# xqtr/PySpecSDR

Hardware: AMD Instinct MI355X
Metric: IQ MSamples/sec end-to-end (FFT+dB+FM demod) (higher is better)
Workload: dtype complex64 IQ / f64 FFT + dB + post-process + FIR + IIR / dB rows stored as f32 / int16 PCM

## Files before the change

pyspecsdr_amd/csrc/pss_fft_r16.h:

```cpp
#pragma once
#include <hip/hip_runtime.h>

#include "pss_npf32.h"
#include "pss_device.h"

namespace pss_r16 {

#ifdef PSS_EXP_NOFMA
__device__ __forceinline__ double2 cmul(double2 a, double2 b) { return make_double2(a.x * b.x - a.y * b.y, a.x * b.y + a.y * b.x); }
__device__ __forceinline__ double power_of(double2 X) { return X.x * X.x + X.y * X.y + 1e-10; }
#else
__device__ __forceinline__ double2 cmul(double2 a, double2 b) { return make_double2(fma(a.x, b.x, -(a.y * b.y)), fma(a.x, b.y, a.y * b.x)); }
__device__ __forceinline__ double power_of(double2 X) { return fma(X.x, X.x, fma(X.y, X.y, 1e-10)); }
#endif
__device__ __forceinline__ double2 cadd(double2 a, double2 b) { return make_double2(a.x + b.x, a.y + b.y); }
__device__ __forceinline__ double2 csub(double2 a, double2 b) { return make_double2(a.x - b.x, a.y - b.y); }

constexpr int brev(int i, int bits)
{
    int r = 0;
    for (int b = 0; b < bits; b++) r |= ((i >> b) & 1) << (bits - 1 - b);
    return r;
}
constexpr int ilog2c(int n) { return n <= 1 ? 0 : 1 + ilog2c(n >> 1); }

template <int J, int LEN>
__device__ __forceinline__ double2 twc(double2 a)
{
    constexpr int j16 = (J * (16 / LEN)) & 15;
    constexpr double C1 = 0.92387953251128673848, S1 = 0.38268343236508978178, H = 0.70710678118654752440;
    if constexpr (j16 == 0) return a;
    else if constexpr (j16 == 4) return make_double2(a.y, -a.x);
    else if constexpr (j16 == 8) return make_double2(-a.x, -a.y);
    else if constexpr (j16 == 12) return make_double2(-a.y, a.x);
    else if constexpr (j16 == 2) return make_double2((a.x + a.y) * H, (a.y - a.x) * H);
    else if constexpr (j16 == 6) return make_double2((a.y - a.x) * H, -(a.x + a.y) * H);
    else if constexpr (j16 == 1) return cmul(a, make_double2(C1, -S1));
    else if constexpr (j16 == 3) return cmul(a, make_double2(S1, -C1));
    else if constexpr (j16 == 5) return cmul(a, make_double2(-S1, -C1));
    else if constexpr (j16 == 7) return cmul(a, make_double2(-C1, -S1));
    else return a;
}

template <int R, int LEN = R, int BASE = 0>
struct Dif {
    template <int J>
    static __device__ __forceinline__ void bf(double2 (&v)[R])
    {
        if constexpr (J < LEN / 2) {
            double2 a = v[BASE + J], b = v[BASE + J + LEN / 2];
            v[BASE + J] = cadd(a, b);
            v[BASE + J + LEN / 2] = twc<J, LEN>(csub(a, b));
            bf<J + 1>(v);
        }
    }
    static __device__ __forceinline__ void run(double2 (&v)[R])
    {
        if constexpr (LEN >= 2) {
            bf<0>(v);
            Dif<R, LEN / 2, BASE>::run(v);
            Dif<R, LEN / 2, BASE + LEN / 2>::run(v);
        }
    }
};

template <int R>
__device__ __forceinline__ void fft_reg(double2 (&v)[R])
{
    if constexpr (R > 1) Dif<R>::run(v);
}

static __constant__ double2 DB_TAB[97] = {
    {0x1.5555555555555p+0, -0x1.ffbfc2bbc7802p-4},
    {0x1.51d07eae2f815p+0, -0x1.ed50a4a26eafbp-4},
    {0x1.4e5e0a72f0539p+0, -0x1.db11ed766abf2p-4},
    {0x1.4afd6a052bf5bp+0, -0x1.c902a19e65114p-4},
    {0x1.47ae147ae147bp+0, -0x1.b721cd17157e3p-4},
    {0x1.446f86562d9fbp+0, -0x1.a56e8325f5c87p-4},
    {0x1.4141414141414p+0, -0x1.93e7de0fc3e7fp-4},
    {0x1.3e22cbce4a902p+0, -0x1.828cfed29a212p-4},
    {0x1.3b13b13b13b14p+0, -0x1.715d0ce367afdp-4},
    {0x1.3813813813814p+0, -0x1.605735ee985f4p-4},
    {0x1.3521cfb2b78c1p+0, -0x1.4f7aad9bbcbaep-4},
    {0x1.323e34a2b10bfp+0, -0x1.3ec6ad5407866p-4},
    {0x1.2f684bda12f68p+0, -0x1.2e3a740b7800dp-4},
    {0x1.2c9fb4d812ca0p+0, -0x1.1dd5460c8b170p-4},
    {0x1.29e4129e4129ep+0, -0x1.0d966cc6500f8p-4},
    {0x1.27350b8812735p+0, -0x1.fafa6d397efdbp-5},
    {0x1.2492492492492p+0, -0x1.db11ed766abf1p-5},
    {0x1.21fb78121fb78p+0, -0x1.bb7209d1e24e4p-5},
    {0x1.1f7047dc11f70p+0, -0x1.9c197abf00dd3p-5},
    {0x1.1cf06ada2811dp+0, -0x1.7d070145f4fd8p-5},
    {0x1.1a7b9611a7b96p+0, -0x1.5e3966b7e9294p-5},
    {0x1.1811811811812p+0, -0x1.3faf7c6630614p-5},
    {0x1.15b1e5f75270dp+0, -0x1.21681b5c8c213p-5},
    {0x1.135c81135c811p+0, -0x1.0362241e638eap-5},
    {0x1.1111111111111p+0, -0x1.cb38fccd8bfdap-6},
    {0x1.0ecf56be69c90p+0, -0x1.902c31d62a847p-6},
    {0x1.0c9714fbcda3bp+0, -0x1.559bd2406c3c1p-6},
    {0x1.0a6810a6810a7p+0, -0x1.1b85d6044e9bbp-6},
    {0x1.0842108421084p+0, -0x1.c3d0837784c3ap-7},
    {0x1.0624dd2f1a9fcp+0, -0x1.51824c7587eb5p-7},
    {0x1.0410410410410p+0, -0x1.c03a80ae5e038p-8},
    {0x1.0204081020408p+0, -0x1.be76bd77b4fb5p-9},
    {0x1.0000000000000p+0, 0x0.0p+0},
    {0x1.fc07f01fc07f0p-1, 0x1.bafd47221ed34p-9},
    {0x1.f81f81f81f820p-1, 0x1.b9476a4fcd0f3p-8},
    {0x1.f44659e4a4271p-1, 0x1.49b085144368ep-7},
    {0x1.f07c1f07c1f08p-1, 0x1.b5e908eb13789p-7},
    {0x1.ecc07b301ecc0p-1, 0x1.10a83a8446c7fp-6},
    {0x1.e9131abf0b767p-1, 0x1.45f4f5acb8be3p-6},
    {0x1.e573ac901e574p-1, 0x1.7adc3df3b1ff3p-6},
    {0x1.e1e1e1e1e1e1ep-1, 0x1.af5f92b00e611p-6},
    {0x1.de5d6e3f8868ap-1, 0x1.e3806acbd0593p-6},
    {0x1.dae6076b981dbp-1, 0x1.0ba01a816ffffp-5},
    {0x1.d77b654b82c34p-1, 0x1.25502c0fc3148p-5},
    {0x1.d41d41d41d41dp-1, 0x1.3ed1199a5e427p-5},
    {0x1.d0cb58f6ec074p-1, 0x1.58238eeb353dcp-5},
    {0x1.cd85689039b0bp-1, 0x1.71483427d2a97p-5},
    {0x1.ca4b3055ee191p-1, 0x1.8a3fadeb847f4p-5},
    {0x1.c71c71c71c71cp-1, 0x1.a30a9d609efedp-5},
    {0x1.c3f8f01c3f8f0p-1, 0x1.bba9a058dfd85p-5},
    {0x1.c0e070381c0e0p-1, 0x1.d41d5164facb7p-5},
    {0x1.bdd2b899406f7p-1, 0x1.ec6647eb5880bp-5},
    {0x1.bacf914c1bad0p-1, 0x1.02428c1f08014p-4},
    {0x1.b7d6c3dda338bp-1, 0x1.0e3d29d81165fp-4},
    {0x1.b4e81b4e81b4fp-1, 0x1.1a23445501814p-4},
    {0x1.b2036406c80d9p-1, 0x1.25f5215eb594ap-4},
    {0x1.af286bca1af28p-1, 0x1.31b3055c4711ap-4},
    {0x1.ac5701ac5701bp-1, 0x1.3d5d335c53178p-4},
    {0x1.a98ef606a63bep-1, 0x1.48f3ed1df48f9p-4},
    {0x1.a6d01a6d01a6dp-1, 0x1.5477731973e85p-4},
    {0x1.a41a41a41a41ap-1, 0x1.5fe80488af4fep-4},
    {0x1.a16d3f97a4b02p-1, 0x1.6b45df6f3e2c8p-4},
    {0x1.9ec8e951033d9p-1, 0x1.769140a2526fdp-4},
    {0x1.9c2d14ee4a102p-1, 0x1.81ca63d05a448p-4},
    {0x1.999999999999ap-1, 0x1.8cf183886480bp-4},
    {0x1.970e4f80cb872p-1, 0x1.9806d9414a20cp-4},
    {0x1.948b0fcd6e9e0p-1, 0x1.a30a9d609efebp-4},
    {0x1.920fb49d0e229p-1, 0x1.adfd07416be06p-4},
    {0x1.8f9c18f9c18fap-1, 0x1.b8de4d3ab3d97p-4},
    {0x1.8d3018d3018d3p-1, 0x1.c3aea4a5c6effp-4},
    {0x1.8acb90f6bf3aap-1, 0x1.ce6e41e463da3p-4},
    {0x1.886e5f0abb04ap-1, 0x1.d91d5866aa99ap-4},
    {0x1.8618618618618p-1, 0x1.e3bc1ab0e1a00p-4},
    {0x1.83c977ab2beddp-1, 0x1.ee4aba610f205p-4},
    {0x1.8181818181818p-1, 0x1.f8c9683468191p-4},
    {0x1.7f405fd017f40p-1, 0x1.019c2a064b487p-3},
    {0x1.7d05f417d05f4p-1, 0x1.06cbd67a6c3b7p-3},
    {0x1.7ad2208e0ecc3p-1, 0x1.0bf3d0937c41dp-3},
    {0x1.78a4c8178a4c8p-1, 0x1.11142f0811357p-3},
    {0x1.767dce434a9b1p-1, 0x1.162d082ac9d10p-3},
    {0x1.745d1745d1746p-1, 0x1.1b3e71ec94f7ap-3},
    {0x1.724287f46debcp-1, 0x1.204881dee8777p-3},
    {0x1.702e05c0b8170p-1, 0x1.254b4d35e7d3dp-3},
    {0x1.6e1f76b4337c7p-1, 0x1.2a46e8ca7ba29p-3},
    {0x1.6c16c16c16c17p-1, 0x1.2f3b691c5a000p-3},
    {0x1.6a13cd1537290p-1, 0x1.3428e2540096ep-3},
    {0x1.6816816816817p-1, 0x1.390f6844a0b82p-3},
    {0x1.661ec6a5122f9p-1, 0x1.3def0e6dfdf85p-3},
    {0x1.642c8590b2164p-1, 0x1.42c7e7fe3fc02p-3},
    {0x1.623fa77016240p-1, 0x1.479a07d3b6410p-3},
    {0x1.6058160581606p-1, 0x1.4c65807e93337p-3},
    {0x1.5e75bb8d015e7p-1, 0x1.512a644296c3ep-3},
    {0x1.5c9882b931057p-1, 0x1.55e8c518b10f9p-3},
    {0x1.5ac056b015ac0p-1, 0x1.5aa0b4b0988fap-3},
    {0x1.58ed2308158edp-1, 0x1.5f52447255c93p-3},
    {0x1.571ed3c506b3ap-1, 0x1.63fd857fc49bap-3},
    {0x1.5555555555555p-1, 0x1.68a288b60b7fdp-3}};

__device__ __forceinline__ double db64_of_exact(double pw, const double2 *tab = DB_TAB)
{
    const unsigned hi = (unsigned)__double2hiint(pw), lo = (unsigned)__double2loint(pw);
    const bool up = (hi & 0xfffffu) >= 0x80000u;
    const int e = (int)(hi >> 20) - 1023 + (up ? 1 : 0);
    const double z = __hiloint2double((int)((hi & 0xfffffu) | (up ? 0x3fe00000u : 0x3ff00000u)), (int)lo);
    const int i = (int)fma(z, 128.0, -95.5);
    const double2 tc = tab[i];
    const double r = fma(z, tc.x, -1.0);
    double p = fma(r, -0x1.5555555555555p-3, 0x1.999999999999ap-3);
    p = fma(p, r, -0.25);
    p = fma(p, r, 0x1.5555555555555p-2);
    p = fma(p, r, -0.5);
    p = fma(p, r, 1.0);
    double res = fma(p * r, 0x1.bcb7b1526e50ep-2, tc.y);
    res = fma((double)e, 0x1.34413509f79ffp-2, res);
    return hi >= 0x7ff00000u ? pw : 10.0 * res;
}

__device__ __forceinline__ float db_of_exact(double pw, const double2 *tab = DB_TAB)
{
    const unsigned hi = (unsigned)__double2hiint(pw), lo = (unsigned)__double2loint(pw);
    const bool up = (hi & 0xfffffu) >= 0x80000u;
    const int e = (int)(hi >> 20) - 1023 + (up ? 1 : 0);
    const double z = __hiloint2double((int)((hi & 0xfffffu) | (up ? 0x3fe00000u : 0x3ff00000u)), (int)lo);
    const int i = (int)fma(z, 128.0, -95.5);
    const double2 tc = tab[i];
    const double r = fma(z, tc.x, -1.0);
    double p = fma(r, -0x1.5555555555555p-3, 0x1.999999999999ap-3);
    p = fma(p, r, -0.25);
    p = fma(p, r, 0x1.5555555555555p-2);
    p = fma(p, r, -0.5);
    p = fma(p, r, 1.0);
    double res = fma(p * r, 0x1.bcb7b1526e50ep-2, tc.y);
    res = fma((double)e, 0x1.34413509f79ffp-2, res);
    const float out = (float)(10.0 * res);
    return hi >= 0x7ff00000u ? (float)pw : out;
}

__device__ __forceinline__ float db_of_fast(double pw)
{
    const float t = (float)(pw - 1.0);
    const float far = 3.0102999566398120f * __log2f((float)pw);
    const float s = t * __builtin_amdgcn_rcpf(2.0f + t);
    const float s2 = s * s;
#ifdef PSS_EXP_NOFMA
    const float p = s * (2.0f + s2 * (0.66666667f + s2 * (0.4f + s2 * (0.28571429f + s2 * 0.22222222f))));
#else
    const float p = s * fmaf(s2, fmaf(s2, fmaf(s2, fmaf(s2, 0.22222222f, 0.28571429f), 0.4f), 0.66666667f), 2.0f);
#endif
    return fabsf(t) < 0.25f ? 4.342944819032518f * p : far;
}

constexpr int FLAG_SCAN_EXACT = 1, FLAG_DB_EXACT = 2;
__device__ __forceinline__ float db_of(double pw, int flags = 0, const double2 *tab = DB_TAB)
{
    return (flags & FLAG_DB_EXACT) ? db_of_exact(pw, tab) : db_of_fast(pw);
}

typedef unsigned v2u_t __attribute__((ext_vector_type(2)));
__device__ __forceinline__ __amdgpu_buffer_rsrc_t make_rsrc(const void *p, unsigned bytes)
{
    return __builtin_amdgcn_make_buffer_rsrc(const_cast<void *>(p), 0, (int)bytes, 0x00020000);
}
__device__ __forceinline__ float2 buf_load_f2(__amdgpu_buffer_rsrc_t r, int voff, int soff)
{
    const v2u_t v = __builtin_amdgcn_raw_buffer_load_b64(r, voff, soff, 0);
    return make_float2(__uint_as_float(v.x), __uint_as_float(v.y));
}
__device__ __forceinline__ double buf_load_f64(__amdgpu_buffer_rsrc_t r, int voff, int soff)
{
    const v2u_t v = __builtin_amdgcn_raw_buffer_load_b64(r, voff, soff, 0);
    return __hiloint2double((int)v.y, (int)v.x);
}
__device__ __forceinline__ void buf_store_f32(__amdgpu_buffer_rsrc_t r, int voff, int soff, float x)
{
    __builtin_amdgcn_raw_buffer_store_b32(__float_as_uint(x), r, voff, soff, 0);
}
__device__ __forceinline__ void buf_store_f64(__amdgpu_buffer_rsrc_t r, int voff, int soff, double x)
{
    v2u_t v;
    v.x = (unsigned)__double2loint(x);
    v.y = (unsigned)__double2hiint(x);
    __builtin_amdgcn_raw_buffer_store_b64(v, r, voff, soff, 0);
}

constexpr int DPP_NEXT_LANE = 0x134;

template <int LOG_R3>
struct Cfg {
    static constexpr int R3 = 1 << LOG_R3;
    static constexpr int T = 16 * R3;
    static constexpr int N = 16 * T;
    static constexpr int FPW = 256 / T;
#ifdef PSS_EXP_OLDPAD
    static constexpr int E1_STRIDE = T + 4;
    static constexpr int E2_STRIDE = 256 + 2;
    static constexpr int TW2S = 16;
#else
    static constexpr int E1_STRIDE = T + (R3 == 1 ? 4 : R3 % 16);
    static constexpr int E2_STRIDE = 256 + (R3 == 1 ? 2 : R3 <= 8 ? 8 / R3 : 1);
    static constexpr int TW2S = 17;
#endif
    static constexpr int TW2 = R3 * TW2S;
    static __device__ __forceinline__ int tw2_slot(int i) { return (i / 16) * TW2S + (i % 16); }
    static constexpr int EX = (16 * E1_STRIDE > R3 * E2_STRIDE) ? 16 * E1_STRIDE : R3 * E2_STRIDE;
    static constexpr size_t LDS = (size_t)FPW * EX * sizeof(double2) + (size_t)TW2 * sizeof(double2);
};

template <bool WAVE_LOCAL>
__device__ __forceinline__ void frame_sync()
{
    if constexpr (WAVE_LOCAL) {
        __builtin_amdgcn_fence(__ATOMIC_RELEASE, "wavefront");
        __builtin_amdgcn_wave_barrier();
        __builtin_amdgcn_fence(__ATOMIC_ACQUIRE, "wavefront");
    } else {
        __syncthreads();
    }
}

template <int LOG_R3, bool WAVE_LOCAL = false, class Emit>
__device__ __forceinline__ void r16_core(double2 (&v)[16], double2 *ex, const double2 (&tw1)[16], const double2 *tw2,
                                         int t, Emit emit)
{
    using C = Cfg<LOG_R3>;
    constexpr int R3 = C::R3, T = C::T;
    const int k2s = t / R3, m1s = t % R3;
    fft_reg<16>(v);
#pragma unroll
    for (int k2 = 0; k2 < 16; k2++) {
        double2 y = v[brev(k2, 4)];
        if (k2) y = cmul(y, tw1[k2]);
        ex[k2 * C::E1_STRIDE + t] = y;
    }
    frame_sync<WAVE_LOCAL>();
#pragma unroll
    for (int m2 = 0; m2 < 16; m2++) v[m2] = ex[k2s * C::E1_STRIDE + m1s + R3 * m2];
    frame_sync<WAVE_LOCAL>();
#ifndef PSS_EXP_TW2_AT_USE
    constexpr int TWD = 4;
    const double2 *twp = tw2 + m1s * C::TW2S;
    double2 tq[TWD];
    if constexpr (R3 > 1) {
#pragma unroll
        for (int d = 0; d < TWD; d++) tq[d] = twp[1 + d];
        __builtin_amdgcn_sched_barrier(0);
    }
#endif
    fft_reg<16>(v);
#ifdef PSS_EXP_TW2_AT_USE
#pragma unroll
    for (int j2 = 0; j2 < 16; j2++) {
        double2 z = v[brev(j2, 4)];
        if (R3 > 1) z = cmul(z, tw2[m1s * C::TW2S + j2]);
        ex[m1s * C::E2_STRIDE + 16 * j2 + k2s] = z;
    }
#else
    {
#pragma unroll
        for (int j2 = 0; j2 < 16; j2++) {
            double2 z = v[brev(j2, 4)];
            if constexpr (R3 > 1) {
                if (j2 >= 1) {
                    z = cmul(z, tq[(j2 - 1) % TWD]);
                    if (j2 + TWD < 16) tq[(j2 - 1) % TWD] = twp[j2 + TWD];
                }
            }
            ex[m1s * C::E2_STRIDE + 16 * j2 + k2s] = z;
        }
    }
#endif
    frame_sync<WAVE_LOCAL>();
#pragma unroll
    for (int c = 0; c < 16 / R3; c++) {
        double2 b[R3];
#pragma unroll
        for (int m1 = 0; m1 < R3; m1++) b[m1] = ex[m1 * C::E2_STRIDE + t + T * c];
        fft_reg<R3>(b);
#pragma unroll
        for (int j1 = 0; j1 < R3; j1++) emit(c * R3 + j1, 256 * j1 + t + T * c, b[brev(j1, LOG_R3)]);
    }
}

template <int LOG_R3, bool WAVE_LOCAL = false, class Emit>
__device__ __forceinline__ void r16_core_split(double2 (&v)[16], double *ex, const double2 (&tw1)[16], const double2 *tw2,
                                               int t, Emit emit)
{
    using C = Cfg<LOG_R3>;
    constexpr int R3 = C::R3, T = C::T;
    const int k2s = t / R3, m1s = t % R3;
    fft_reg<16>(v);
    double2 y[16];
#pragma unroll
    for (int k2 = 0; k2 < 16; k2++) {
        y[k2] = v[brev(k2, 4)];
        if (k2) y[k2] = cmul(y[k2], tw1[k2]);
    }
#pragma unroll
    for (int k2 = 0; k2 < 16; k2++) ex[k2 * C::E1_STRIDE + t] = y[k2].x;
    frame_sync<WAVE_LOCAL>();
#pragma unroll
    for (int m2 = 0; m2 < 16; m2++) v[m2].x = ex[k2s * C::E1_STRIDE + m1s + R3 * m2];
    frame_sync<WAVE_LOCAL>();
#pragma unroll
    for (int k2 = 0; k2 < 16; k2++) ex[k2 * C::E1_STRIDE + t] = y[k2].y;
    frame_sync<WAVE_LOCAL>();
#pragma unroll
    for (int m2 = 0; m2 < 16; m2++) v[m2].y = ex[k2s * C::E1_STRIDE + m1s + R3 * m2];
    frame_sync<WAVE_LOCAL>();
    fft_reg<16>(v);
#pragma unroll
    for (int j2 = 0; j2 < 16; j2++) {
        y[j2] = v[brev(j2, 4)];
        if (R3 > 1) y[j2] = cmul(y[j2], tw2[m1s * C::TW2S + j2]);
    }
#pragma unroll
    for (int j2 = 0; j2 < 16; j2++) ex[m1s * C::E2_STRIDE + 16 * j2 + k2s] = y[j2].x;
    frame_sync<WAVE_LOCAL>();
#pragma unroll
    for (int c = 0; c < 16 / R3; c++)
#pragma unroll
        for (int m1 = 0; m1 < R3; m1++) v[c * R3 + m1].x = ex[m1 * C::E2_STRIDE + t + T * c];
    frame_sync<WAVE_LOCAL>();
#pragma unroll
    for (int j2 = 0; j2 < 16; j2++) ex[m1s * C::E2_STRIDE + 16 * j2 + k2s] = y[j2].y;
    frame_sync<WAVE_LOCAL>();
#pragma unroll
    for (int c = 0; c < 16 / R3; c++)
#pragma unroll
        for (int m1 = 0; m1 < R3; m1++) v[c * R3 + m1].y = ex[m1 * C::E2_STRIDE + t + T * c];
#pragma unroll
    for (int c = 0; c < 16 / R3; c++) {
        double2 b[R3];
#pragma unroll
        for (int m1 = 0; m1 < R3; m1++) b[m1] = v[c * R3 + m1];
        fft_reg<R3>(b);
#pragma unroll
        for (int j1 = 0; j1 < R3; j1++) emit(c * R3 + j1, 256 * j1 + t + T * c, b[brev(j1, LOG_R3)]);
    }
}

template <int LOG_R3, bool SCAN, bool SPLIT = false, bool PREFETCH = false, bool EXACT = false, bool ONE = false, bool D64 = false>
__global__ __launch_bounds__(256) void k_spectrum_r16(const float2 *__restrict__ iq, float *__restrict__ db,
                                                      const double2 *__restrict__ tw, const double *__restrict__ win,
                                                      long n_frames, float *__restrict__ peak, double *__restrict__ bw,
                                                      int *__restrict__ count, double bin_hz, int flags)
{
    using C = Cfg<LOG_R3>;
    constexpr int R3 = C::R3, T = C::T, N = C::N, FPW = ONE ? 1 : C::FPW;
    static_assert(!ONE || (T >= 128 && !SCAN && !SPLIT), "one frame per workgroup: compute_fft rows of frames of >= 2 wavefronts");
    static_assert(!D64 || (EXACT && !SCAN), "float64 rows: compute_fft rows by the float64 evaluation");
    constexpr int OB = D64 ? 8 : 4;
    extern __shared__ __align__(16) unsigned char smem[];
    double2 *ex_all = reinterpret_cast<double2 *>(smem);
    double2 *tw2 = SPLIT ? reinterpret_cast<double2 *>(smem + (size_t)FPW * C::EX * sizeof(double))
                         : ex_all + (size_t)FPW * C::EX;
    __shared__ float red_f[4];
    __shared__ int red_i[4];
    __shared__ uint4 l10[SCAN ? 16 : 1];
    const int tid = threadIdx.x;
    if (SCAN && tid < 16) l10[tid] = pss::L10_PACK[tid];
    const int fl = tid / T;
    const int t = tid % T;
    double2 *ex = ex_all + (size_t)fl * C::EX;
    double2 tw1[16];
    double w[16];
    tw1[0] = make_double2(1.0, 0.0);
#pragma unroll
    for (int k2 = 1; k2 < 16; k2++) tw1[k2] = tw[(size_t)t * k2];
#pragma unroll
    for (int n2 = 0; n2 < 16; n2++) w[n2] = SCAN ? 1.0 : win[t + T * n2];
    if (tid < R3 * 16) {
        const int m1 = tid / 16, j2 = tid % 16;
        tw2[C::tw2_slot(tid)] = tw[(size_t)(m1 * j2) * 16];
    }
    __syncthreads();
    const long groups = (n_frames + FPW - 1) / FPW;
    float2 nx[16];
    auto fetch = [&](long g) {
        const long f = g * FPW + fl;
#ifdef PSS_EXP_SPEC_L2IQ
        const float2 *x = iq + (size_t)(f < n_frames ? (f & 15) : 0) * N;
#else
        const float2 *x = iq + (size_t)(f < n_frames ? f : 0) * N;
#endif
#pragma unroll
        for (int n2 = 0; n2 < 16; n2++) nx[n2] = x[t + T * n2];
    };
    if (PREFETCH && (long)blockIdx.x < groups) fetch(blockIdx.x);
    for (long g = blockIdx.x; g < groups; g += gridDim.x) {
        const long f = g * FPW + fl;
        const bool valid = f < n_frames;
        double2 v[16];
        if constexpr (!PREFETCH) fetch(g);
#pragma unroll
        for (int n2 = 0; n2 < 16; n2++) v[n2] = make_double2((double)nx[n2].x * w[n2], (double)nx[n2].y * w[n2]);
        if (PREFETCH && g + gridDim.x < groups) fetch(g + gridDim.x);
        float *out = (!PREFETCH && db && valid) ? db + (size_t)f * N * (OB / 4) : nullptr;
        const long f_first = g * FPW;
        const long rows_here = n_frames - f_first < FPW ? n_frames - f_first : FPW;
        const __amdgpu_buffer_rsrc_t ro = make_rsrc((PREFETCH && db) ? db + (size_t)f_first * N * (OB / 4) : nullptr, (PREFETCH && db) ? (unsigned)(rows_here * N * OB) : 0u);
        const int ro_lane = (fl * N + t) * OB;
        float lmax = -INFINITY;
        float dbv[16];
        auto emit = [&](int i, int k, double2 X) {
            if constexpr (D64) {
                const double d64 = db64_of_exact(power_of(X));
                if constexpr (PREFETCH) buf_store_f64(ro, ro_lane, (((k - t) + N / 2) & (N - 1)) * 8, d64);
                else if (out) reinterpret_cast<double *>(out)[(k + N / 2) & (N - 1)] = d64;
                return;
            }
            float d;
            if constexpr (SCAN) d = (flags & FLAG_SCAN_EXACT) ? pss::scan_db_np(X.x, X.y, l10) : db_of_fast(power_of(X));
            else d = EXACT ? db_of_exact(power_of(X)) : db_of_fast(power_of(X));
#ifdef PSS_EXP_SPEC_NODB
            d = (float)X.x + (float)X.y;
#endif
            if constexpr (PREFETCH) buf_store_f32(ro, ro_lane, (((k - t) + N / 2) & (N - 1)) * 4, d);
            else if (out) out[(k + N / 2) & (N - 1)] = d;
            dbv[i] = d;
            lmax = fmaxf(lmax, d);
        };
        constexpr bool WL = T <= 64;
        if (SPLIT) r16_core_split<LOG_R3, WL>(v, reinterpret_cast<double *>(smem) + (size_t)fl * C::EX, tw1, tw2, t, emit);
        else r16_core<LOG_R3, WL>(v, ex, tw1, tw2, t, emit);
        if (SCAN) {
            float m = lmax;
            for (int off = (T < 64 ? T : 64) / 2; off > 0; off >>= 1) m = fmaxf(m, __shfl_xor(m, off));
            if (T > 64) {
                if ((tid & 63) == 0) red_f[tid >> 6] = m;
                __syncthreads();
                m = red_f[(fl * T) >> 6];
                for (int wv = 1; wv < T / 64; wv++) m = fmaxf(m, red_f[((fl * T) >> 6) + wv]);
            }
            const float thr = m - 20.0f;
            int cnt = 0;
#pragma unroll
            for (int i = 0; i < 16; i++) cnt += dbv[i] > thr;
            for (int off = (T < 64 ? T : 64) / 2; off > 0; off >>= 1) cnt += __shfl_xor(cnt, off);
            if (T > 64) {
                if ((tid & 63) == 0) red_i[tid >> 6] = cnt;
                __syncthreads();
                cnt = 0;
                for (int wv = 0; wv < T / 64; wv++) cnt += red_i[((fl * T) >> 6) + wv];
            }
            if (valid && t == 0) {
                peak[f] = m;
                if (bw) bw[f] = (double)cnt * bin_hz;
                if (count) count[f] = cnt;
            }
        }
        frame_sync<T <= 64 && !SCAN>();
    }
}

template <int LOG_R, bool WINDOW>
__global__ __launch_bounds__(256) void k_spectrum_r16_big(const float2 *__restrict__ iq, float *__restrict__ db,
                                                          const double2 *__restrict__ tw, const double *__restrict__ win,
                                                          long n_frames, double2 *__restrict__ scratch, int flags)
{
    using C = Cfg<4>;
    constexpr int T = C::T, NS = C::N, R = 1 << LOG_R, N = R * NS;
    extern __shared__ __align__(16) unsigned char smem[];
    double2 *ex = reinterpret_cast<double2 *>(smem);
    double2 *tw2 = ex + C::EX;
    const int t = threadIdx.x;
    double2 *scr = scratch + (size_t)blockIdx.x * N;
    double2 tw1[16];
    tw1[0] = make_double2(1.0, 0.0);
#pragma unroll
    for (int k2 = 1; k2 < 16; k2++) tw1[k2] = tw[(size_t)t * k2 * R];
    tw2[C::tw2_slot(t)] = tw[(size_t)((t / 16) * (t % 16)) * 16 * R];
    __syncthreads();
    for (long f = blockIdx.x; f < n_frames; f += gridDim.x) {
        const float2 *x = iq + (size_t)f * N;
        float *out = db + (size_t)f * N;
#pragma unroll 4
        for (int j = 0; j < 16; j++) {
            const int n = t + T * j;
            double2 a[R];
#pragma unroll
            for (int q = 0; q < R; q++) {
                float2 s = x[n + NS * q];
                const double wv = WINDOW ? win[n + NS * q] : 1.0;
                a[q] = make_double2((double)s.x * wv, (double)s.y * wv);
            }
            fft_reg<R>(a);
#pragma unroll
            for (int r = 0; r < R; r++) {
                double2 y = a[brev(r, LOG_R)];
                if (r) y = cmul(y, tw[(size_t)n * r]);
                scr[(size_t)r * NS + n] = y;
            }
        }
        __syncthreads();
        for (int r = 0; r < R; r++) {
            double2 v[16];
#pragma unroll
            for (int n2 = 0; n2 < 16; n2++) v[n2] = scr[(size_t)r * NS + t + T * n2];
            r16_core<4>(v, ex, tw1, tw2, t, [&](int, int kp, double2 X) {
                const int k = R * kp + r;
                out[(k + N / 2) & (N - 1)] = db_of(power_of(X), flags);
            });
            __syncthreads();
        }
    }
}

template <int LOG_R, class Load, class Store>
__global__ __launch_bounds__(256) void k_big_g(Load load, Store store, const double2 *__restrict__ tw, long n_frames,
                                               double2 *__restrict__ scratch)
{
    using C = Cfg<4>;
    constexpr int T = C::T, NS = C::N, R = 1 << LOG_R, N = R * NS;
    extern __shared__ __align__(16) unsigned char smem[];
    double2 *ex = reinterpret_cast<double2 *>(smem);
    double2 *tw2 = ex + C::EX;
    const int t = threadIdx.x;
    double2 *scr = scratch + (size_t)blockIdx.x * N;
    double2 tw1[16];
    tw1[0] = make_double2(1.0, 0.0);
#pragma unroll
    for (int k2 = 1; k2 < 16; k2++) tw1[k2] = tw[(size_t)t * k2 * R];
    tw2[C::tw2_slot(t)] = tw[(size_t)((t / 16) * (t % 16)) * 16 * R];
    __syncthreads();
    for (long f = blockIdx.x; f < n_frames; f += gridDim.x) {
#pragma unroll 2
        for (int j = 0; j < 16; j++) {
            const int n = t + T * j;
            double2 a[R];
#pragma unroll
            for (int q = 0; q < R; q++) a[q] = load(f, (size_t)(n + NS * q));
            fft_reg<R>(a);
#pragma unroll
            for (int r = 0; r < R; r++) {
                double2 y = a[brev(r, LOG_R)];
                if (r) y = cmul(y, tw[(size_t)n * r]);
                scr[(size_t)r * NS + n] = y;
            }
        }
        __syncthreads();
        for (int r = 0; r < R; r++) {
            double2 v[16];
#pragma unroll
            for (int n2 = 0; n2 < 16; n2++) v[n2] = scr[(size_t)r * NS + t + T * n2];
            r16_core<4>(v, ex, tw1, tw2, t, [&](int, int kp, double2 X) { store(f, (size_t)(R * kp + r), X); });
            __syncthreads();
        }
    }
}

__global__ __launch_bounds__(256) void k_huge_p1(const float2 *__restrict__ iq, const double2 *__restrict__ tw,
                                                 const double *__restrict__ win, double2 *__restrict__ Y, int NS, long n_frames)
{
    using C = Cfg<0>;
    constexpr int EXP = C::EX + 1;
    extern __shared__ __align__(16) unsigned char smem[];
    double2 *ex_all = reinterpret_cast<double2 *>(smem);
    const int tid = threadIdx.x, fl = tid & 15, t = tid >> 4;
    const size_t N = (size_t)256 * NS;
    const int cpf = NS / 16;
    double2 tw1[16];
    tw1[0] = make_double2(1.0, 0.0);
#pragma unroll
    for (int k2 = 1; k2 < 16; k2++) tw1[k2] = tw[(size_t)(t * k2) * NS];
    double2 *ex = ex_all + (size_t)fl * EXP;
    const long total = n_frames * cpf;
    for (long g = blockIdx.x; g < total; g += gridDim.x) {
        const long f = g / cpf;
        const int col = (int)(g - f * cpf) * 16 + fl;
        const float2 *x = iq + (size_t)f * N;
        double2 v[16];
#pragma unroll
        for (int j = 0; j < 16; j++) {
            const size_t idx = (size_t)col + (size_t)NS * (t + 16 * j);
            const float2 sv = x[idx];
            const double wv = win[idx];
            v[j] = make_double2((double)sv.x * wv, (double)sv.y * wv);
        }
        double2 *Yf = Y + (size_t)f * N;
        r16_core<0>(v, ex, tw1, nullptr, t, [&](int, int r, double2 X) {
            if (r) X = cmul(X, tw[(size_t)col * r]);
            Yf[(size_t)r * NS + col] = X;
        });
        __syncthreads();
    }
}

template <int LOG_R3>
__global__ __launch_bounds__(256) void k_huge_p2(const double2 *__restrict__ Y, float *__restrict__ db,
                                                 const double2 *__restrict__ tw, long n_rows, int flags)
{
    using C = Cfg<LOG_R3>;
    constexpr int R3 = C::R3, T = C::T, NS = C::N, FPW = C::FPW;
    extern __shared__ __align__(16) unsigned char smem[];
    double2 *ex_all = reinterpret_cast<double2 *>(smem);
    double2 *tw2 = ex_all + (size_t)FPW * C::EX;
    const int tid = threadIdx.x, fl = tid / T, t = tid % T;
    double2 *ex = ex_all + (size_t)fl * C::EX;
    const size_t N = (size_t)256 * NS;
    double2 tw1[16];
    tw1[0] = make_double2(1.0, 0.0);
#pragma unroll
    for (int k2 = 1; k2 < 16; k2++) tw1[k2] = tw[(size_t)(t * k2) * 256];
    if (tid < R3 * 16) {
        const int m1 = tid / 16, j2 = tid % 16;
        tw2[C::tw2_slot(tid)] = tw[(size_t)(m1 * j2) * 16 * 256];
    }
    __syncthreads();
    const long groups = (n_rows + FPW - 1) / FPW;
    for (long g = blockIdx.x; g < groups; g += gridDim.x) {
        const long row = g * FPW + fl;
        const long f = row >> 8;
        const int r = (int)(row & 255);
        const double2 *y = Y + (size_t)row * NS;
        double2 v[16];
#pragma unroll
        for (int n2 = 0; n2 < 16; n2++) v[n2] = y[t + T * n2];
        float *out = db + (size_t)f * N;
        r16_core<LOG_R3>(v, ex, tw1, tw2, t, [&](int, int kp, double2 X) {
            const size_t k = (size_t)256 * kp + r;
            out[(k + N / 2) & (N - 1)] = db_of(power_of(X), flags);
        });
        __syncthreads();
    }
}

template <class Load>
__global__ __launch_bounds__(256) void k_huge_p1_g(Load load, const double2 *__restrict__ tw, double2 *__restrict__ Y, int NS,
                                                   long n_frames)
{
    using C = Cfg<0>;
    constexpr int EXP = C::EX + 1;
    extern __shared__ __align__(16) unsigned char smem[];
    double2 *ex_all = reinterpret_cast<double2 *>(smem);
    const int tid = threadIdx.x, fl = tid & 15, t = tid >> 4;
    const size_t N = (size_t)256 * NS;
    const int cpf = NS / 16;
    double2 tw1[16];
    tw1[0] = make_double2(1.0, 0.0);
#pragma unroll
    for (int k2 = 1; k2 < 16; k2++) tw1[k2] = tw[(size_t)(t * k2) * NS];
    double2 *ex = ex_all + (size_t)fl * EXP;
    const long total = n_frames * cpf;
    for (long g = blockIdx.x; g < total; g += gridDim.x) {
        const long f = g / cpf;
        const int col = (int)(g - f * cpf) * 16 + fl;
        double2 v[16];
#pragma unroll
        for (int j = 0; j < 16; j++) v[j] = load(f, (size_t)col + (size_t)NS * (t + 16 * j));
        double2 *Yf = Y + (size_t)f * N;
        r16_core<0>(v, ex, tw1, nullptr, t, [&](int, int r, double2 X) {
            if (r) X = cmul(X, tw[(size_t)col * r]);
            Yf[(size_t)r * NS + col] = X;
        });
        __syncthreads();
    }
}

template <int LOG_R3, class Store>
__global__ __launch_bounds__(256) void k_huge_p2_g(const double2 *__restrict__ Y, Store store, const double2 *__restrict__ tw,
                                                   long n_rows)
{
    using C = Cfg<LOG_R3>;
    constexpr int R3 = C::R3, T = C::T, NS = C::N, FPW = C::FPW;
    extern __shared__ __align__(16) unsigned char smem[];
    double2 *ex_all = reinterpret_cast<double2 *>(smem);
    double2 *tw2 = ex_all + (size_t)FPW * C::EX;
    const int tid = threadIdx.x, fl = tid / T, t = tid % T;
    double2 *ex = ex_all + (size_t)fl * C::EX;
    double2 tw1[16];
    tw1[0] = make_double2(1.0, 0.0);
#pragma unroll
    for (int k2 = 1; k2 < 16; k2++) tw1[k2] = tw[(size_t)(t * k2) * 256];
    if (tid < R3 * 16) {
        const int m1 = tid / 16, j2 = tid % 16;
        tw2[C::tw2_slot(tid)] = tw[(size_t)(m1 * j2) * 16 * 256];
    }
    __syncthreads();
    const long groups = (n_rows + FPW - 1) / FPW;
    for (long g = blockIdx.x; g < groups; g += gridDim.x) {
        const long row = g * FPW + fl;
        const long f = row >> 8;
        const int r = (int)(row & 255);
        const double2 *y = Y + (size_t)row * NS;
        double2 v[16];
#pragma unroll
        for (int n2 = 0; n2 < 16; n2++) v[n2] = y[t + T * n2];
        r16_core<LOG_R3>(v, ex, tw1, tw2, t, [&](int, int kp, double2 X) { store(f, (size_t)256 * kp + r, X); });
        __syncthreads();
    }
}

}
```

pyspecsdr_amd/csrc/pss_fft_xl.h:

```cpp
#pragma once
#include <hip/hip_runtime.h>

#include "pss_fft_r16.h"

namespace pss_xl {

using pss_r16::brev;
using pss_r16::cmul;
using pss_r16::fft_reg;

template <int LOG_R4>
struct CfgX {
    static constexpr int R4 = 1 << LOG_R4;
    static constexpr int T = 256 * R4;
    static constexpr int N = 16 * T;
    static constexpr int T2 = 16 * R4;
    static constexpr int E2 = T2 + R4;
#ifdef PSS_EXP_OLDPAD
    static constexpr int P3 = 16 * 272 + 32 / R4;
#else
    static constexpr int P3 = 16 * 272 + 16 / R4;
#endif
    static constexpr int EXD = (R4 * P3 > 256 * E2) ? R4 * P3 : 256 * E2;
    static constexpr size_t LDS = (size_t)EXD * sizeof(double);
};

__device__ __forceinline__ void twiddle_powers(double2 (&v)[16], double2 w)
{
    const double2 w2 = cmul(w, w);
    double2 po = w, pe = w2;
    v[brev(1, 4)] = cmul(v[brev(1, 4)], po);
    v[brev(2, 4)] = cmul(v[brev(2, 4)], pe);
#pragma unroll
    for (int j = 1; j < 7; j++) {
        po = cmul(po, w2);
        pe = cmul(pe, w2);
        v[brev(2 * j + 1, 4)] = cmul(v[brev(2 * j + 1, 4)], po);
        v[brev(2 * j + 2, 4)] = cmul(v[brev(2 * j + 2, 4)], pe);
    }
    po = cmul(po, w2);
    v[brev(15, 4)] = cmul(v[brev(15, 4)], po);
}

using pss_r16::v2u_t;
using pss_r16::make_rsrc;
using pss_r16::buf_load_f2;
using pss_r16::buf_load_f64;
using pss_r16::buf_store_f32;

__device__ __forceinline__ void sched_fence() { asm volatile("" ::: "memory"); }

template <bool WAVE_LOCAL = false>
__device__ __forceinline__ void xsync()
{
    if constexpr (WAVE_LOCAL) {
        __builtin_amdgcn_fence(__ATOMIC_RELEASE, "wavefront");
        __builtin_amdgcn_wave_barrier();
        __builtin_amdgcn_fence(__ATOMIC_ACQUIRE, "wavefront");
    } else {
        __syncthreads();
    }
}
template <bool WAVE_LOCAL = false, class Wr, class Rd>
__device__ __forceinline__ void exchange(double2 (&v)[16], Wr wr, Rd rd)
{
    double im[16];
#pragma unroll
    for (int i = 0; i < 16; i++) { *wr(i) = v[brev(i, 4)].x; im[i] = v[brev(i, 4)].y; }
    xsync<WAVE_LOCAL>();
#pragma unroll
    for (int i = 0; i < 16; i++) v[i].x = *rd(i);
    xsync<WAVE_LOCAL>();
#pragma unroll
    for (int i = 0; i < 16; i++) *wr(i) = im[i];
    xsync<WAVE_LOCAL>();
#pragma unroll
    for (int i = 0; i < 16; i++) v[i].y = *rd(i);
    xsync<WAVE_LOCAL>();
}

template <int LOG_R4, class Emit>
__device__ __forceinline__ void xl_core(double2 (&v)[16], double *ex, double2 w1, double2 w2, double2 w3, int t, Emit emit)
{
    using C = CfgX<LOG_R4>;
    constexpr int R4 = C::R4, T = C::T, T2 = C::T2, E2 = C::E2, P3 = C::P3;
    const int r_s = t / T2, b_s = t % T2;
    const int g3 = t / R4, c_s = t % R4;
    fft_reg<16>(v);
    twiddle_powers(v, w1);
    {
        double *w_lo = ex + t, *w_hi = ex + 8 * T + t;
        double *rb = ex + r_s * T + b_s;
        exchange(v, [&](int r) { return (r < 8 ? w_lo : w_hi) + (r & 7) * T; }, [&](int q) { return rb + T2 * q; });
    }
    fft_reg<16>(v);
    twiddle_powers(v, w2);
    {
        double *wb = ex + (r_s * 16) * E2 + b_s, *rb = ex + g3 * E2 + c_s;
#ifdef PSS_EXP_XL_BARRIERS
        exchange(v, [&](int r2) { return wb + r2 * E2; }, [&](int q) { return rb + R4 * q; });
#else
        exchange<true>(v, [&](int r2) { return wb + r2 * E2; }, [&](int q) { return rb + R4 * q; });
        __syncthreads();
#endif
    }
    fft_reg<16>(v);
    if constexpr (R4 > 1) twiddle_powers(v, w3);
    {
        double *wb = ex + c_s * P3 + 17 * (g3 & 15) + (g3 >> 4);
        double *rb0 = ex + 272 * (t >> 8) + 17 * ((t >> 4) & 15) + (t & 15);
        double *rb1 = rb0 + (R4 > 2 ? 2 * P3 : 0);
        exchange(v, [&](int r3) { return wb + 272 * r3; },
                 [&](int i) { return ((i % R4) < 2 ? rb0 : rb1) + ((i % R4) & 1) * P3 + 272 * R4 * (i / R4); });
    }
#pragma unroll
    for (int j = 0; j < 16 / R4; j++) {
        double2 b[R4];
#pragma unroll
        for (int k = 0; k < R4; k++) b[k] = v[j * R4 + k];
        fft_reg<R4>(b);
#pragma unroll
        for (int k = 0; k < R4; k++) emit(j * R4 + k, j, k, b[brev(k, LOG_R4)]);
    }
}

template <int LOG_R4, bool WINDOW, bool SCAN = false, bool EXACT = false>
__global__ __launch_bounds__(256 << LOG_R4, 4) void k_spectrum_xl(const float2 *__restrict__ iq, float *__restrict__ db,
                                                                  const double2 *__restrict__ tw, const double *__restrict__ win,
                                                                  long n_frames, float *__restrict__ peak, double *__restrict__ bw,
                                                                  int *__restrict__ count, double bin_hz, int flags)
{
    using C = CfgX<LOG_R4>;
    constexpr int T = C::T, N = C::N, T2 = C::T2, R4 = C::R4;
    extern __shared__ __align__(16) unsigned char smem[];
    __shared__ float red_f[16];
    __shared__ int red_i[16];
    __shared__ uint4 l10[SCAN ? 16 : 1];
    double *ex = reinterpret_cast<double *>(smem);
    const int t = threadIdx.x;
    if (SCAN && t < 16) l10[t] = pss::L10_PACK[t];
    if (SCAN) __syncthreads();
    const double2 w1 = tw[t];
    const double2 w2 = tw[(size_t)(t % T2) * 16];
    const double2 w3 = tw[(size_t)(t % R4) * 256];
    const __amdgpu_buffer_rsrc_t rw = make_rsrc(win, WINDOW ? N * 8 : 0);
    for (long f = blockIdx.x; f < n_frames; f += gridDim.x) {
#ifdef PSS_EXP_SPEC_L2IQ
        const __amdgpu_buffer_rsrc_t rx = make_rsrc(iq + (size_t)(f & 15) * N, N * 8);
#else
        const __amdgpu_buffer_rsrc_t rx = make_rsrc(iq + (size_t)f * N, N * 8);
#endif
#ifdef PSS_EXP_SPEC_NOSTORE
        const __amdgpu_buffer_rsrc_t ro = make_rsrc(db + (size_t)f * N, (flags & 0x100) ? N * 4 : 0);
#else
        const __amdgpu_buffer_rsrc_t ro = make_rsrc(db ? db + (size_t)f * N : nullptr, db ? N * 4 : 0);
#endif
        double2 u1 = w1, u2 = w2, u3 = w3;
        asm volatile("" : "+v"(u1.x), "+v"(u1.y), "+v"(u2.x), "+v"(u2.y), "+v"(u3.x), "+v"(u3.y));
        double2 v[16];
#pragma unroll
        for (int h = 0; h < 2; h++) {
            float2 s[8];
            double wv[8];
#pragma unroll
            for (int q = 0; q < 8; q++) s[q] = buf_load_f2(rx, t * 8, T * (8 * h + q) * 8);
#pragma unroll
            for (int q = 0; q < 8; q++) wv[q] = WINDOW ? buf_load_f64(rw, t * 8, T * (8 * h + q) * 8) : 1.0;
#pragma unroll
            for (int q = 0; q < 8; q++) v[8 * h + q] = make_double2((double)s[q].x * wv[q], (double)s[q].y * wv[q]);
            sched_fence();
        }
        float lmax = -INFINITY;
        float *held = reinterpret_cast<float *>(ex);
        xl_core<LOG_R4>(v, ex, u1, u2, u3, t, [&](int i, int j, int k, double2 X) {
            float d;
            if constexpr (SCAN) d = (flags & pss_r16::FLAG_SCAN_EXACT) ? pss::scan_db_np(X.x, X.y, l10) : pss_r16::db_of_fast(pss_r16::power_of(X));
            else d = EXACT ? pss_r16::db_of_exact(pss_r16::power_of(X)) : pss_r16::db_of_fast(pss_r16::power_of(X));
#ifdef PSS_EXP_SPEC_NODB
            d = (float)X.x + (float)X.y;
#endif
            buf_store_f32(ro, t * 4, ((4096 * k + T * j + N / 2) & (N - 1)) * 4, d);
            if (SCAN) { held[i * T + t] = d; lmax = fmaxf(lmax, d); }
        });
        if (SCAN) {
            float m = lmax;
            for (int off = 32; off > 0; off >>= 1) m = fmaxf(m, __shfl_xor(m, off));
            if ((t & 63) == 0) red_f[t >> 6] = m;
            __syncthreads();
            m = red_f[0];
#pragma unroll
            for (int wv = 1; wv < T / 64; wv++) m = fmaxf(m, red_f[wv]);
            const float thr = m - 20.0f;
            int cnt = 0;
#pragma unroll
            for (int i = 0; i < 16; i++) cnt += held[i * T + t] > thr;
            for (int off = 32; off > 0; off >>= 1) cnt += __shfl_xor(cnt, off);
            if ((t & 63) == 0) red_i[t >> 6] = cnt;
            __syncthreads();
            if (t == 0) {
                cnt = 0;
                for (int wv = 0; wv < T / 64; wv++) cnt += red_i[wv];
                peak[f] = m;
                if (bw) bw[f] = (double)cnt * bin_hz;
                if (count) count[f] = cnt;
            }
        }
    }
}

}
```

pyspecsdr_amd/csrc/pss_spec_post.h:

```cpp
#pragma once

namespace pss_sp {

using namespace pss_r16;

#ifndef PSS_EXP_FUSE_WAVES
#define PSS_EXP_FUSE_WAVES 2
#endif
template <bool ROW32, bool ROW64>
__global__ __launch_bounds__(256, PSS_EXP_FUSE_WAVES) void k_spectrum_post(const float2 *__restrict__ iq, float *__restrict__ db32, double *__restrict__ db64,
                                                       const double2 *__restrict__ tw, const double *__restrict__ win, long n_frames,
                                                       double *__restrict__ row_lo, double *__restrict__ row_hi, double *__restrict__ vals,
                                                       int disp_w)
{
    using C = Cfg<2>;
    constexpr int R3 = C::R3, T = C::T, N = C::N, FPW = C::FPW;
    static_assert(T == 64, "a frame is one wavefront");
    constexpr int EPL = 16;
    using PC = pss_post::PostCfg<EPL, double>;
    static_assert((size_t)(T + 1) * PC::S * sizeof(double) <= (size_t)C::EX * sizeof(double2), "the staged row fits the frame's exchange buffer");
    extern __shared__ __align__(16) unsigned char smem[];
    double2 *ex_all = reinterpret_cast<double2 *>(smem);
#ifdef PSS_EXP_FUSE_LDS
    constexpr size_t EXS = PSS_EXP_FUSE_LDS / FPW / sizeof(double2);
    double2 *tw2 = ex_all;
#else
    constexpr size_t EXS = C::EX;
    double2 *tw2 = ex_all + (size_t)FPW * C::EX;
#endif
#ifdef PSS_EXP_POST_PRIO
    __builtin_amdgcn_s_setprio(PSS_EXP_POST_PRIO);
#endif
    const int tid = threadIdx.x;
    const int fl = __builtin_amdgcn_readfirstlane(tid / T);
    const int t = tid % T;
    double2 *ex = ex_all + (size_t)fl * EXS;
    double *stage = reinterpret_cast<double *>(ex);
    double2 tw1[16];
    double w[16];
    tw1[0] = make_double2(1.0, 0.0);
#pragma unroll
    for (int k2 = 1; k2 < 16; k2++) tw1[k2] = tw[(size_t)t * k2];
#pragma unroll
    for (int n2 = 0; n2 < 16; n2++) w[n2] = win[t + T * n2];
#ifndef PSS_EXP_FUSE_LDS
    if (tid < R3 * 16) {
        const int m1 = tid / 16, j2 = tid % 16;
        tw2[C::tw2_slot(tid)] = tw[(size_t)(m1 * j2) * 16];
    }
#endif
    __syncthreads();
    const long groups = (n_frames + FPW - 1) / FPW;
    float2 nx[16];
    auto fetch = [&](long g) {
        const long f = g * FPW + fl;
        const float2 *x = iq + (size_t)(f < n_frames ? f : 0) * N;
#pragma unroll
        for (int n2 = 0; n2 < 16; n2++) nx[n2] = x[t + T * n2];
    };
    if ((long)blockIdx.x < groups) fetch(blockIdx.x);
    int phase = 0;
    for (long g = blockIdx.x; g < groups; g += gridDim.x) {
        const long f = g * FPW + fl;
        const bool valid = f < n_frames;
        double2 v[16];
#pragma unroll
#ifdef PSS_EXP_FUSE_NOFFT
        for (int n2 = 0; n2 < 16; n2++) v[n2] = make_double2((double)nx[n2].x, (double)nx[n2].y);
#else
        for (int n2 = 0; n2 < 16; n2++) v[n2] = make_double2((double)nx[n2].x * w[n2], (double)nx[n2].y * w[n2]);
#endif
        if (g + gridDim.x < groups) fetch(g + gridDim.x);
        const long f_first = g * FPW;
        const long rows_here = n_frames - f_first < FPW ? n_frames - f_first : FPW;
        const __amdgpu_buffer_rsrc_t ro32 = make_rsrc((ROW32 && db32) ? db32 + (size_t)f_first * N : nullptr, (ROW32 && db32) ? (unsigned)(rows_here * N * 4) : 0u);
        const __amdgpu_buffer_rsrc_t ro64 = make_rsrc((ROW64 && db64) ? db64 + (size_t)f_first * N : nullptr, (ROW64 && db64) ? (unsigned)(rows_here * N * 8) : 0u);
        const int lane_el = fl * N + t;
        double dbv[16];
        auto emit = [&](int i, int k, double2 X) {
            const double d64 = db64_of_exact(power_of(X));
            const int e0 = ((k - t) + N / 2) & (N - 1);
            if constexpr (ROW64) buf_store_f64(ro64, lane_el * 8, e0 * 8, d64);
            if constexpr (ROW32) buf_store_f32(ro32, lane_el * 4, e0 * 4, (float)d64);
            dbv[i] = d64;
        };
#ifdef PSS_EXP_FUSE_NOFFT
#pragma unroll
        for (int i = 0; i < 16; i++) emit(i, 256 * (i % R3) + t + T * (i / R3), v[i]);
#else
        r16_core<2, true>(v, ex, tw1, tw2, t, emit);
#endif
        frame_sync<true>();
#pragma unroll
        for (int i = 0; i < 16; i++) {
            const int c = i / R3, j1 = i % R3;
            const int e = (((256 * j1 + T * c) + N / 2) & (N - 1)) + t;
            stage[(e / EPL) * PC::S + (e % EPL)] = dbv[i];
        }
        frame_sync<true>();
#ifndef PSS_EXP_FUSE_NOPOST
        if (valid) {
            int slot[PC::Q];
#pragma unroll
            for (int j = 0; j < PC::Q; j++) slot[j] = 0;
            pss_post::post_row_staged<EPL, 1, true, double>(stage, slot, t, N - 4, nullptr, fl, t, phase, nullptr, row_lo, row_hi, f, nullptr, vals, disp_w);
        }
#endif
        frame_sync<true>();
    }
#ifdef PSS_EXP_POST_PRIO
    __builtin_amdgcn_s_setprio(0);
#endif
}

}
```

Measured before the change: 69680.

## Stage dB table in LDS, buffer-load IQ, defer row stores after FFT

Copies the 97-entry dB lookup table from constant memory into shared memory in the spectrum kernels and passes it to the exact dB evaluators. The fused spectrum+post kernel now loads IQ with buffer loads whose range is zero for out-of-range frames, which drops the branch guards. It also moves the dB row stores out of the FFT emit callback into a separate loop after the FFT, and precomputes a per-lane staging pointer. The aim is to avoid scalar/constant-cache pressure from divergent table lookups and to cut address arithmetic, at the cost of extra LDS, an added barrier in the xl kernel, and more live registers.

```diff
diff --git a/pyspecsdr_amd/csrc/pss_fft_r16.h b/pyspecsdr_amd/csrc/pss_fft_r16.h
--- a/pyspecsdr_amd/csrc/pss_fft_r16.h
+++ b/pyspecsdr_amd/csrc/pss_fft_r16.h
@@ -70,7 +70,8 @@
     if constexpr (R > 1) Dif<R>::run(v);
 }
 
-static __constant__ double2 DB_TAB[97] = {
+constexpr int DB_TAB_N = 97;
+static __constant__ double2 DB_TAB[DB_TAB_N] = {
     {0x1.5555555555555p+0, -0x1.ffbfc2bbc7802p-4},
     {0x1.51d07eae2f815p+0, -0x1.ed50a4a26eafbp-4},
     {0x1.4e5e0a72f0539p+0, -0x1.db11ed766abf2p-4},
@@ -429,8 +430,10 @@
     __shared__ float red_f[4];
     __shared__ int red_i[4];
     __shared__ uint4 l10[SCAN ? 16 : 1];
+    __shared__ double2 dbt[EXACT ? DB_TAB_N : 1];
     const int tid = threadIdx.x;
     if (SCAN && tid < 16) l10[tid] = pss::L10_PACK[tid];
+    if (EXACT && tid < DB_TAB_N) dbt[tid] = DB_TAB[tid];
     const int fl = tid / T;
     const int t = tid % T;
     double2 *ex = ex_all + (size_t)fl * C::EX;
@@ -476,14 +479,14 @@
         float dbv[16];
         auto emit = [&](int i, int k, double2 X) {
             if constexpr (D64) {
-                const double d64 = db64_of_exact(power_of(X));
+                const double d64 = db64_of_exact(power_of(X), dbt);
                 if constexpr (PREFETCH) buf_store_f64(ro, ro_lane, (((k - t) + N / 2) & (N - 1)) * 8, d64);
                 else if (out) reinterpret_cast<double *>(out)[(k + N / 2) & (N - 1)] = d64;
                 return;
             }
             float d;
             if constexpr (SCAN) d = (flags & FLAG_SCAN_EXACT) ? pss::scan_db_np(X.x, X.y, l10) : db_of_fast(power_of(X));
-            else d = EXACT ? db_of_exact(power_of(X)) : db_of_fast(power_of(X));
+            else d = EXACT ? db_of_exact(power_of(X), dbt) : db_of_fast(power_of(X));
 #ifdef PSS_EXP_SPEC_NODB
             d = (float)X.x + (float)X.y;
 #endif
diff --git a/pyspecsdr_amd/csrc/pss_fft_xl.h b/pyspecsdr_amd/csrc/pss_fft_xl.h
--- a/pyspecsdr_amd/csrc/pss_fft_xl.h
+++ b/pyspecsdr_amd/csrc/pss_fft_xl.h
@@ -136,13 +136,15 @@
     __shared__ float red_f[16];
     __shared__ int red_i[16];
     __shared__ uint4 l10[SCAN ? 16 : 1];
+    __shared__ double2 dbt[EXACT ? pss_r16::DB_TAB_N : 1];
     double *ex = reinterpret_cast<double *>(smem);
     const int t = threadIdx.x;
     if (SCAN && t < 16) l10[t] = pss::L10_PACK[t];
-    if (SCAN) __syncthreads();
     const double2 w1 = tw[t];
     const double2 w2 = tw[(size_t)(t % T2) * 16];
     const double2 w3 = tw[(size_t)(t % R4) * 256];
+    if (EXACT && t < pss_r16::DB_TAB_N) dbt[t] = pss_r16::DB_TAB[t];
+    if (SCAN || EXACT) __syncthreads();
     const __amdgpu_buffer_rsrc_t rw = make_rsrc(win, WINDOW ? N * 8 : 0);
     for (long f = blockIdx.x; f < n_frames; f += gridDim.x) {
 #ifdef PSS_EXP_SPEC_L2IQ
@@ -175,7 +177,7 @@
         xl_core<LOG_R4>(v, ex, u1, u2, u3, t, [&](int i, int j, int k, double2 X) {
             float d;
             if constexpr (SCAN) d = (flags & pss_r16::FLAG_SCAN_EXACT) ? pss::scan_db_np(X.x, X.y, l10) : pss_r16::db_of_fast(pss_r16::power_of(X));
-            else d = EXACT ? pss_r16::db_of_exact(pss_r16::power_of(X)) : pss_r16::db_of_fast(pss_r16::power_of(X));
+            else d = EXACT ? pss_r16::db_of_exact(pss_r16::power_of(X), dbt) : pss_r16::db_of_fast(pss_r16::power_of(X));
 #ifdef PSS_EXP_SPEC_NODB
             d = (float)X.x + (float)X.y;
 #endif
diff --git a/pyspecsdr_amd/csrc/pss_spec_post.h b/pyspecsdr_amd/csrc/pss_spec_post.h
--- a/pyspecsdr_amd/csrc/pss_spec_post.h
+++ b/pyspecsdr_amd/csrc/pss_spec_post.h
@@ -20,6 +20,7 @@
     using PC = pss_post::PostCfg<EPL, double>;
     static_assert((size_t)(T + 1) * PC::S * sizeof(double) <= (size_t)C::EX * sizeof(double2), "the staged row fits the frame's exchange buffer");
     extern __shared__ __align__(16) unsigned char smem[];
+    __shared__ double2 dbt[DB_TAB_N];
     double2 *ex_all = reinterpret_cast<double2 *>(smem);
 #ifdef PSS_EXP_FUSE_LDS
     constexpr size_t EXS = PSS_EXP_FUSE_LDS / FPW / sizeof(double2);
@@ -36,6 +37,7 @@
     const int t = tid % T;
     double2 *ex = ex_all + (size_t)fl * EXS;
     double *stage = reinterpret_cast<double *>(ex);
+    double *st_lane = stage + (t / EPL) * PC::S + t % EPL;
     double2 tw1[16];
     double w[16];
     tw1[0] = make_double2(1.0, 0.0);
@@ -49,16 +51,17 @@
         tw2[C::tw2_slot(tid)] = tw[(size_t)(m1 * j2) * 16];
     }
 #endif
+    if (tid < DB_TAB_N) dbt[tid] = DB_TAB[tid];
     __syncthreads();
     const long groups = (n_frames + FPW - 1) / FPW;
     float2 nx[16];
     auto fetch = [&](long g) {
         const long f = g * FPW + fl;
-        const float2 *x = iq + (size_t)(f < n_frames ? f : 0) * N;
+        const __amdgpu_buffer_rsrc_t rx = make_rsrc(iq + (size_t)(f < n_frames ? f : 0) * N, f < n_frames ? N * 8 : 0);
 #pragma unroll
-        for (int n2 = 0; n2 < 16; n2++) nx[n2] = x[t + T * n2];
+        for (int n2 = 0; n2 < 16; n2++) nx[n2] = buf_load_f2(rx, t * 8, T * n2 * 8);
     };
-    if ((long)blockIdx.x < groups) fetch(blockIdx.x);
+    fetch(blockIdx.x);
     int phase = 0;
     for (long g = blockIdx.x; g < groups; g += gridDim.x) {
         const long f = g * FPW + fl;
@@ -70,32 +73,33 @@
 #else
         for (int n2 = 0; n2 < 16; n2++) v[n2] = make_double2((double)nx[n2].x * w[n2], (double)nx[n2].y * w[n2]);
 #endif
-        if (g + gridDim.x < groups) fetch(g + gridDim.x);
+        fetch(g + gridDim.x);
         const long f_first = g * FPW;
         const long rows_here = n_frames - f_first < FPW ? n_frames - f_first : FPW;
         const __amdgpu_buffer_rsrc_t ro32 = make_rsrc((ROW32 && db32) ? db32 + (size_t)f_first * N : nullptr, (ROW32 && db32) ? (unsigned)(rows_here * N * 4) : 0u);
         const __amdgpu_buffer_rsrc_t ro64 = make_rsrc((ROW64 && db64) ? db64 + (size_t)f_first * N : nullptr, (ROW64 && db64) ? (unsigned)(rows_here * N * 8) : 0u);
         const int lane_el = fl * N + t;
         double dbv[16];
-        auto emit = [&](int i, int k, double2 X) {
-            const double d64 = db64_of_exact(power_of(X));
-            const int e0 = ((k - t) + N / 2) & (N - 1);
-            if constexpr (ROW64) buf_store_f64(ro64, lane_el * 8, e0 * 8, d64);
-            if constexpr (ROW32) buf_store_f32(ro32, lane_el * 4, e0 * 4, (float)d64);
-            dbv[i] = d64;
-        };
+        auto emit = [&](int i, int k, double2 X) { dbv[i] = db64_of_exact(power_of(X), dbt); };
 #ifdef PSS_EXP_FUSE_NOFFT
 #pragma unroll
         for (int i = 0; i < 16; i++) emit(i, 256 * (i % R3) + t + T * (i / R3), v[i]);
 #else
         r16_core<2, true>(v, ex, tw1, tw2, t, emit);
 #endif
+#pragma unroll
+        for (int i = 0; i < 16; i++) {
+            const int c = i / R3, j1 = i % R3;
+            const int e0 = ((256 * j1 + T * c) + N / 2) & (N - 1);
+            if constexpr (ROW64) buf_store_f64(ro64, lane_el * 8, e0 * 8, dbv[i]);
+            if constexpr (ROW32) buf_store_f32(ro32, lane_el * 4, e0 * 4, (float)dbv[i]);
+        }
         frame_sync<true>();
 #pragma unroll
         for (int i = 0; i < 16; i++) {
             const int c = i / R3, j1 = i % R3;
-            const int e = (((256 * j1 + T * c) + N / 2) & (N - 1)) + t;
-            stage[(e / EPL) * PC::S + (e % EPL)] = dbv[i];
+            const int e0 = ((256 * j1 + T * c) + N / 2) & (N - 1);
+            st_lane[(e0 / EPL) * PC::S] = dbv[i];
         }
         frame_sync<true>();
 #ifndef PSS_EXP_FUSE_NOPOST
```

After: 70370 (median of 6 runs). No clear change (+1.0%).
